# jaronlong52/neuron_poker

Hardware: AMD Instinct MI355X
Metric: Monte Carlo hand evals/sec @100k iters, 6-max preflop (higher is better)
Workload: dtype u32

## Files before the change

### neuron_poker_amd/csrc/mcq_device.hpp

```cpp
#pragma once
#include <stdint.h>

#include <algorithm>
#include <vector>

#include "../../include/mcq.h"

#if defined(__HIPCC__)
#include <hip/hip_runtime.h>
#define MCQ_HD __host__ __device__ __forceinline__
#define MCQ_HDM __host__ __device__ __forceinline__
#else
#define MCQ_HD static inline
#define MCQ_HDM inline
#endif

#define MCQ_STREAM_ITERS 16u
#define MCQ_WAVE 64u
#define MCQ_TASK_ITERS (MCQ_STREAM_ITERS * MCQ_WAVE)
#define MCQ_MAX_OPP 9

MCQ_HD uint32_t mcq_popc(uint32_t x) {
#if defined(__HIP_DEVICE_COMPILE__)
    return (uint32_t)__popc(x);
// ... 593 lines not shown
    for (uint32_t r = 0; r < MCQ_SUM_ROWS; r++) order[r] = r;
    std::stable_sort(order.begin(), order.end(), [&](uint32_t a, uint32_t b) {
        return row_lo[a + 1u] - row_lo[a] > row_lo[b + 1u] - row_lo[b];
    });
    std::vector<uint32_t> nxt(MCQ_SUM_SLOTS + 1u);
    for (uint32_t i = 0; i <= MCQ_SUM_SLOTS; i++) nxt[i] = i;
    auto next_free = [&](uint32_t i) -> uint32_t {
        while (nxt[i] != i) {
            nxt[i] = nxt[nxt[i]];
            i = nxt[i];
        }
        return i;
    };
    for (uint32_t i = 0; i < 256u; i++) t->sum.sel8[i] = t->sel8[i];
    for (uint32_t i = 0; i < MCQ_SUM_ROWS; i++) t->sum.hoff[i] = 0;
    for (uint32_t i = 0; i < MCQ_SUM_SLOTS; i++) t->sum.hrank[i] = 0;
    for (uint32_t oi = 0; oi < MCQ_SUM_ROWS && ok; oi++) {
        const uint32_t r = order[oi], lo = row_lo[r], hi = row_lo[r + 1u];
        if (lo == hi) break;
        const uint32_t col0 = MCQ_SUM_COL(ms[lo].sum), col1 = MCQ_SUM_COL(ms[hi - 1u].sum);
        uint32_t d = 0;
        for (;; d++) {
            const uint32_t at = next_free(d + col0 < MCQ_SUM_SLOTS ? d + col0 : MCQ_SUM_SLOTS);
            d = at - col0;
            if (d + col1 >= MCQ_SUM_SLOTS || d > 0xFFFFu) { ok = false; break; }
            bool fits = true;
            for (uint32_t k = lo + 1u; k < hi && fits; k++) fits = t->sum.hrank[d + MCQ_SUM_COL(ms[k].sum)] == 0u;
            if (fits) break;
        }
        if (!ok) break;
        t->sum.hoff[r] = (uint16_t)d;
        for (uint32_t k = lo; k < hi; k++) {
            const uint32_t slot = d + MCQ_SUM_COL(ms[k].sum);
            nxt[slot] = slot + 1u;
            t->sum.hrank[slot] = (uint16_t)id_of(ms[k].key);
        }
    }
    return ok;
}
static inline void mcq_fill_sum_tables(McqTables *t) { (void)mcq_fill_sum_tables_checked(t, nullptr); }

struct McqQueryCtx {
    uint32_t deck_lo, deck_hi;
    uint32_t L0;
    uint32_t n_opp;
    uint32_t n_deal;
    uint32_t runs;
    McqHole hero;
    McqBoard board;
    McqSumHole hero_s;
    McqSumBoard board_s;
};

struct McqQueryWords {
    uint32_t w0, w1, w2, w3;
    MCQ_HDM uint32_t card(uint32_t k) const {
        uint64_t v = ((uint64_t)w1 << 32) | w0;
        return (uint32_t)(v >> (8u * k)) & 0xFFu;
    }
    MCQ_HDM uint32_t n_board() const { return w1 >> 24; }
    MCQ_HDM uint32_t n_players() const { return w2 & 0xFFu; }
    MCQ_HDM uint32_t reserved() const { return w2 >> 8; }
    MCQ_HDM uint32_t runs() const { return w3; }
};

MCQ_HD bool mcq_query_valid(const McqQueryWords &q) {
    if (q.n_board() > 5 || q.n_players() < 1 || q.n_players() > 10 || q.reserved() != 0) return false;
    uint64_t seen = 0;
    bool ok = true;
    for (uint32_t i = 0; i < 2u + q.n_board(); i++) {
        uint32_t c = q.card(i);
        ok = ok && c < 52 && !((seen >> (c & 63u)) & 1);
        seen |= 1ull << (c & 63u);
    }
    return ok;
}

MCQ_HD void mcq_query_ctx(const McqQueryWords &q, McqQueryCtx &c) {
    uint64_t deck = (1ull << 52) - 1;
    c.board.clear();
    c.board_s.clear();
    for (uint32_t i = 0; i < q.n_board(); i++) {
        const uint32_t cd = q.card(2u + i);
        deck &= ~(1ull << cd);
        c.board.add(mcq_card(cd));
        c.board_s.add(mcq_card_sum(cd));
    }
    const uint32_t h0 = q.card(0), h1 = q.card(1);
    deck &= ~(1ull << h0);
    deck &= ~(1ull << h1);
    c.hero.set(mcq_card(h0), mcq_card(h1));
    c.hero_s.set(mcq_card_sum(h0), mcq_card_sum(h1));
    c.deck_lo = (uint32_t)deck;
    c.deck_hi = (uint32_t)(deck >> 32);
    c.L0 = 50u - q.n_board();
    c.n_opp = q.n_players() - 1u;
    c.n_deal = 5u - q.n_board();
    c.runs = q.runs();
}

MCQ_HD uint32_t mcq_task_weight(const McqQueryWords &q) {
    const uint32_t n = q.n_players(), deal = 5u - q.n_board();
    return 160u + 200u * n + 10u * n * n + deal * (162u - 9u * n);
}
MCQ_HD uint32_t mcq_task_count(const McqQueryWords &q) {
    return q.runs() / MCQ_TASK_ITERS + (q.runs() % MCQ_TASK_ITERS != 0u ? 1u : 0u);
}

struct McqPart {
    uint32_t t_lo, t_hi, runs;
};
MCQ_HD McqPart mcq_part(uint32_t tasks, uint32_t runs, uint32_t part, uint32_t n_parts) {
    McqPart p;
    p.t_lo = (uint32_t)((uint64_t)tasks * part / n_parts);
    p.t_hi = (uint32_t)((uint64_t)tasks * (part + 1u) / n_parts);
    const uint64_t a = (uint64_t)p.t_lo * MCQ_TASK_ITERS, b = (uint64_t)p.t_hi * MCQ_TASK_ITERS;
    p.runs = (uint32_t)((b < runs ? b : runs) - (a < runs ? a : runs));
    return p;
}

#define MCQ_SPLIT_FROM_PREP 0xFFFFFFFFu
MCQ_HD uint32_t mcq_pick_split(uint64_t total_tasks, uint64_t max_tasks, uint32_t n_cu, uint32_t split_max) {
    const uint64_t want = 8ull * n_cu;
    uint32_t s = 0;
    while (s < split_max && (total_tasks << (s + 1u)) <= want && (max_tasks << (s + 1u)) <= 512u) s++;
    return s;
}

static inline McqQueryWords mcq_query_words(const mcq_query &q) {
    McqQueryWords w;
    __builtin_memcpy(&w, &q, 16);
    return w;
}

MCQ_HD McqCard mcq_base_entry(const McqQueryCtx &qc, uint32_t l, const uint32_t *sel8) {
    uint32_t dlo = qc.deck_lo, dhi = qc.deck_hi;
    uint32_t c = mcq_select_pop(dlo, dhi, l, sel8);
    return mcq_card_sum(c < 52u ? c : 0u);
}

struct McqDeckAoS {
    const McqCard *base128;
    MCQ_HDM McqCard card(uint32_t at) const { return base128[at]; }
    MCQ_HDM McqCard hole_card(uint32_t at) const { return base128[at]; }
};
struct __attribute__((aligned(8))) McqPair {
    uint32_t a, b;
};
template <uint32_t YOFF>
struct McqDeckSplit {
    const McqPair *x128;
    MCQ_HDM McqCard card(uint32_t at) const {
        const McqPair x = x128[at], y = x128[at + YOFF];
        const McqCard c = {x.a, x.b, y.a, y.b};
        return c;
    }
    MCQ_HDM McqCard hole_card(uint32_t at) const {
        const uint32_t rb = x128[at].a;
        const McqPair y = x128[at + YOFF];
        const McqCard c = {rb, 0u, y.a, y.b};
        return c;
    }
    static MCQ_HDM void put(McqPair *x, uint32_t e, const McqCard &c) {
        const McqPair px = {c.rb, c.cnt}, py = {c.los, c.his};
        x[e] = px;
        x[e + YOFF] = py;
    }
};

struct McqLaneAcc {
    static constexpr bool kWays = false, kSeats = false;
    uint64_t types;
    uint32_t tie;
    uint32_t passes;
};
#define MCQ_N_WAYS 9u
struct McqLaneAccWays {
    static constexpr bool kWays = true, kSeats = false;
    uint64_t types;
    uint32_t passes;
    uint64_t ways;
};
#define MCQ_MAX_SEATS 10u
#define MCQ_SEAT_WIN_SHIFT 16u
#define MCQ_SEAT_TIE_SHIFT 21u
struct McqLaneAccSeats {
    static constexpr bool kWays = false, kSeats = true;
    uint32_t passes;
    uint32_t seat[MCQ_MAX_SEATS];
};
static_assert(MCQ_STREAM_ITERS * MCQ_SHARE_UNIT < (1u << MCQ_SEAT_WIN_SHIFT) && MCQ_STREAM_ITERS < 32u, "fields of McqLaneAccSeats");
MCQ_HD uint32_t mcq_seat_increment(uint32_t k) {
    static constexpr uint32_t kInc[MCQ_MAX_SEATS] = {
        2520u | (1u << MCQ_SEAT_WIN_SHIFT), 1260u | (1u << MCQ_SEAT_TIE_SHIFT), 840u | (1u << MCQ_SEAT_TIE_SHIFT),
        630u | (1u << MCQ_SEAT_TIE_SHIFT),  504u | (1u << MCQ_SEAT_TIE_SHIFT),  420u | (1u << MCQ_SEAT_TIE_SHIFT),
        360u | (1u << MCQ_SEAT_TIE_SHIFT),  315u | (1u << MCQ_SEAT_TIE_SHIFT),  280u | (1u << MCQ_SEAT_TIE_SHIFT),
        252u | (1u << MCQ_SEAT_TIE_SHIFT)};
    return kInc[k - 1u];
}

#define MCQ_HOLE_SENTINEL 0x7F7F7F7Fu

MCQ_HD void mcq_hole_reg(uint32_t rb, uint32_t &h, uint32_t &k) {
#ifdef MCQ_ABLATE_HOLES
    k += (rb ^ h) & 1u;
    return;
#endif
    const uint32_t f = ((rb - h) >> 7) & 0x01010101u;
    k = mcq_sad_u8(f, k);
    h = h + f - 0x01010101u;
}

template <int SLOT>
MCQ_HD void mcq_hole_put(uint32_t &h, uint32_t rp) {
    constexpr uint32_t sh = 8u * (SLOT & 3);
#ifdef MCQ_ABLATE_HOLES
    h = mcq_bfi(0x7Fu << sh, rp << sh, h);
    return;
#endif
    h = h + (rp << sh) - ((0x80u + 0x7Fu - (uint32_t)(SLOT & 3)) << sh);
}

MCQ_HD void mcq_hole_pair(uint32_t rp, uint32_t &h, uint32_t &k) {
    const uint32_t rp0 = h;
#ifdef MCQ_ABLATE_HOLES
    k += (rp ^ rp0) & 1u;
    h = (rp << 8) + rp0;
    return;
#endif
    const uint32_t f = rp0 <= rp ? 1u : 0u;
    k = k + f;
    const uint32_t t = mcq_opaque((rp << 8) + rp0);
    uint32_t c = MCQ_HOLE_SENTINEL - 0x01010101u - 0x7E7Eu - 0x8080u - 1u;
#if defined(__HIP_DEVICE_COMPILE__)
    asm("" : "+v"(c));
    unsigned carry_out;
    h = __builtin_addc(t, c, f, &carry_out);
#else
    h = t + c + f;
#endif
}

template <int J>
MCQ_HD uint32_t mcq_draw_opp(uint32_t rp, uint32_t (&H)[5]) {
    uint32_t k = rp;
    if (J % 4 == 1) mcq_hole_pair(rp, H[J / 4], k);
    if (J % 4 == 0) H[J / 4] = rp;
    if (J >= 2) {
        const uint32_t rb = mcq_splat_byte(rp);
#pragma unroll
        for (int i = 0; i < (J % 4 < 2 ? J / 4 : J / 4 + 1); i++) mcq_hole_reg(rb, H[i], k);
        if (J % 4 >= 2) mcq_hole_put<J>(H[J / 4], rp);
    }
    return mcq_opaque(k);
}

MCQ_HD void mcq_hole_count(uint32_t rb, uint32_t h, uint32_t &k) {
#ifdef MCQ_ABLATE_HOLES
    k += (rb ^ h) & 1u;
    return;
#endif
    k = mcq_opaque(mcq_popc((rb - h) & 0x80808080u) + k);
}

template <int K, int NREGS>
MCQ_HD uint32_t mcq_draw_table(uint32_t rp, const uint32_t (&H)[5], uint32_t &hb) {
    uint32_t p = rp;
    if (K == 0) {
        hb = rp;
    } else if (K == 1) {
        mcq_hole_pair(rp, hb, p);
    } else {
        const uint32_t rb = mcq_splat_byte(rp);
        mcq_hole_reg(rb, hb, p);
        if (K < 4) mcq_hole_put<K>(hb, rp);
    }
    uint32_t k = p;
    if (NREGS > 0) {
        const uint32_t pb = mcq_splat_byte(p);
#pragma unroll
        for (int i = 0; i < NREGS; i++) mcq_hole_count(pb, H[i], k);
    }
    return mcq_opaque(k);
}

template <int NREGS, class Draws, int NDEAL = -1, class Deck = McqDeckAoS>
MCQ_HD void mcq_deal_table(const McqQueryCtx &qc, Draws &dr, const Deck &deck, const uint32_t (&H)[5], uint32_t L,
                           McqSumBoard &b) {
    uint32_t hb = MCQ_HOLE_SENTINEL;
    const uint32_t n_deal = NDEAL >= 0 ? (uint32_t)NDEAL : mcq_opaque_uniform(qc.n_deal);
    McqCard pend = {0u, 0u, 0u, 0u};
#define MCQ_TABLE(K)                                                                                            \
    if (K < n_deal) {                                                                                           \
        const uint32_t at = mcq_draw_table<K, NREGS>(dr.template table<K>(L - Draws::kTableShort), H, hb);  \
        if (K > 0) b.add(pend);                                                                                 \
        pend = deck.card(at);                                                                                   \
        L -= 1;                                                                                                 \
    }
    MCQ_TABLE(0) MCQ_TABLE(1) MCQ_TABLE(2) MCQ_TABLE(3) MCQ_TABLE(4)
#undef MCQ_TABLE
    if (n_deal > 0u) b.add(pend);
}

MCQ_HD void mcq_join_hold(McqCard &c) {
#if defined(__HIP_DEVICE_COMPILE__)
    asm volatile("" : "+v"(c.los), "+v"(c.his));
#else
    (void)c;
#endif
}
template <class Draws, int NOPP = -1, int NDEAL = -1, class Acc = McqLaneAcc, class Deck = McqDeckAoS>
MCQ_HD void mcq_iteration_sum(const McqQueryCtx &qc, Draws &dr, const Deck &deck, const McqSumTabs &tabs, Acc &acc) {
    uint32_t H[5] = {MCQ_HOLE_SENTINEL, MCQ_HOLE_SENTINEL, MCQ_HOLE_SENTINEL, MCQ_HOLE_SENTINEL, MCQ_HOLE_SENTINEL};
    uint32_t L = qc.L0;
    McqSumHole opp[MCQ_MAX_OPP];
    const uint32_t n_opp_d = NOPP >= 0 ? (uint32_t)NOPP : mcq_opaque_uniform(qc.n_opp);
    constexpr bool kLate = NOPP >= 1;
    McqCard j1 = {0u, 0u, 0u, 0u}, j2 = {0u, 0u, 0u, 0u};
#define MCQ_OPP(P)                                                                                             \
    if (P < n_opp_d) {                                                                                         \
        uint32_t r1, r2;                                                                                       \
        dr.template pair<P>(L, r1, r2);   \
        const McqCard c1 = deck.hole_card(mcq_draw_opp<2 * P>(r1, H));               \
        const McqCard c2 = deck.hole_card(mcq_draw_opp<2 * P + 1>(r2, H));  \
        if constexpr (kLate) {                                                                                 \
            if (P > 0) {                                                                                       \
                mcq_join_hold(j2);                                                                             \
                opp[P > 0 ? P - 1 : 0].set(j1, j2);                                                            \
            }                                                                                                  \
            j1 = c1;                                                                                           \
            j2 = c2;                                                                                           \
        } else {                                                                                               \
            opp[P].set(c1, c2);                                                                                \
        }                                                                                                      \
        L -= 2;                                                                                                \
    }
    MCQ_OPP(0) MCQ_OPP(1) MCQ_OPP(2) MCQ_OPP(3) MCQ_OPP(4) MCQ_OPP(5) MCQ_OPP(6) MCQ_OPP(7) MCQ_OPP(8)
#undef MCQ_OPP
    McqSumBoard b = qc.board_s;
    if (NDEAL == 5) b.clear();
    if (NOPP >= 0) {
        mcq_deal_table<(NOPP >= 0 ? (2 * NOPP + 3) / 4 : 0), Draws, NDEAL>(qc, dr, deck, H, L, b);
    } else switch (mcq_opaque_uniform((2u * qc.n_opp + 3u) / 4u)) {
        case 0: mcq_deal_table<0, Draws>(qc, dr, deck, H, L, b); break;
        case 1: mcq_deal_table<1, Draws>(qc, dr, deck, H, L, b); break;
        case 2: mcq_deal_table<2, Draws>(qc, dr, deck, H, L, b); break;
        case 3: mcq_deal_table<3, Draws>(qc, dr, deck, H, L, b); break;
        case 4: mcq_deal_table<4, Draws>(qc, dr, deck, H, L, b); break;
        default: mcq_deal_table<5, Draws>(qc, dr, deck, H, L, b); break;
    }
    if constexpr (kLate) {
        mcq_join_hold(j2);
        opp[NOPP >= 1 ? NOPP - 1 : 0].set(j1, j2);
    }
    McqFlushSel fs;
    fs.from_board(b);
    const uint32_t hk = mcq_sum_key(b, fs, qc.hero_s, tabs);
    uint32_t best = 0;
    uint32_t n_equal = 0;
    const uint32_t n_opp_e = NOPP >= 0 ? (uint32_t)NOPP : mcq_opaque_uniform(qc.n_opp);
#define MCQ_EVAL(P)  \
    if (P < n_opp_e) {                                                     \
        uint32_t rid, fid;                                                 \
        mcq_sum_ids(b, fs, opp[P], tabs, rid, fid);                        \
        if (Acc::kWays) {  \
            const uint32_t k = rid > fid ? rid : fid;                      \
            n_equal += k == hk ? 1u : 0u;                                  \
            best = k > best ? k : best;                                    \
        } else {                                                           \
            best = mcq_max3(best, rid, fid);                               \
        }                                                                  \
    }
#ifndef MCQ_ABLATE_EVAL
    if constexpr (NOPP >= 1 && !Acc::kWays) {
        uint32_t s[MCQ_MAX_OPP], d[MCQ_MAX_OPP], fid[MCQ_MAX_OPP], rid[MCQ_MAX_OPP];
#pragma unroll
        for (int P = 0; P < NOPP; P++) mcq_sum_first(b, fs, opp[P], tabs, s[P], d[P], fid[P]);
#pragma unroll
        for (int P = 0; P < NOPP; P++) rid[P] = mcq_sum_rank(tabs, s[P], d[P]);
#pragma unroll
        for (int P = 0; P < NOPP; P++) best = mcq_max3(best, rid[P], fid[P]);
    } else
#endif
    {
        MCQ_EVAL(0) MCQ_EVAL(1) MCQ_EVAL(2) MCQ_EVAL(3) MCQ_EVAL(4) MCQ_EVAL(5) MCQ_EVAL(6) MCQ_EVAL(7) MCQ_EVAL(8)
    }
#undef MCQ_EVAL
    uint64_t won = hk >= best ? 1u : 0u;
    acc.types += won << (6u * (hk >> MCQ_ID_SHIFT));
    if constexpr (Acc::kWays) acc.ways += won << (6u * n_equal);
    else acc.tie += hk == best ? 1u : 0u;
}
template <class Draws, int NOPP = -1, int NDEAL = -1, class Acc = McqLaneAcc>
MCQ_HD void mcq_iteration(const McqQueryCtx &qc, Draws &dr, const McqCard *base128, const uint32_t *tf,
                          const uint32_t *, const uint32_t *, Acc &acc) {
    const McqDeckAoS deck = {base128};
    mcq_iteration_sum<Draws, NOPP, NDEAL, Acc>(qc, dr, deck, mcq_sum_tabs_of(tf), acc);
}

template <bool STRAIGHT, class Draws, class Acc, class Deck>
MCQ_HD void mcq_iterations_sum(const McqQueryCtx &qc, Draws &dr, const Deck &deck, const McqSumTabs &tabs, Acc &acc,
                               uint32_t cnt) {
    if (STRAIGHT) {
#define MCQ_STRAIGHT(N)                                                                                   \
    case N:                                                                                               \
        if (qc.n_deal == 5u)                                                                          \
            for (uint32_t j = 0; j < cnt; j++) mcq_iteration_sum<Draws, N, 5, Acc>(qc, dr, deck, tabs, acc); \
        else if (qc.n_deal == 2u)                                                                         \
            for (uint32_t j = 0; j < cnt; j++) mcq_iteration_sum<Draws, N, 2, Acc>(qc, dr, deck, tabs, acc); \
        else if (qc.n_deal == 1u)                                                                         \
            for (uint32_t j = 0; j < cnt; j++) mcq_iteration_sum<Draws, N, 1, Acc>(qc, dr, deck, tabs, acc); \
        else                                                                                              \
            for (uint32_t j = 0; j < cnt; j++) mcq_iteration_sum<Draws, N, -1, Acc>(qc, dr, deck, tabs, acc); \
        return;
        switch (qc.n_opp) {
            MCQ_STRAIGHT(1) MCQ_STRAIGHT(2) MCQ_STRAIGHT(3) MCQ_STRAIGHT(4) MCQ_STRAIGHT(5) MCQ_STRAIGHT(6) MCQ_STRAIGHT(7)
            case 8:
                for (uint32_t j = 0; j < cnt; j++) mcq_iteration_sum<Draws, 8, -1, Acc>(qc, dr, deck, tabs, acc);
                return;
            case 9:
                for (uint32_t j = 0; j < cnt; j++) mcq_iteration_sum<Draws, 9, -1, Acc>(qc, dr, deck, tabs, acc);
                return;
            default: break;
        }
#undef MCQ_STRAIGHT
    }
    for (uint32_t j = 0; j < cnt; j++) mcq_iteration_sum<Draws, -1, -1, Acc>(qc, dr, deck, tabs, acc);
}
template <bool STRAIGHT, class Draws, class Acc>
MCQ_HD void mcq_iterations(const McqQueryCtx &qc, Draws &dr, const McqCard *base128, const uint32_t *tf, const uint32_t *,
                           const uint32_t *, Acc &acc, uint32_t cnt) {
    const McqDeckAoS deck = {base128};
    mcq_iterations_sum<STRAIGHT>(qc, dr, deck, mcq_sum_tabs_of(tf), acc, cnt);
}

template <class Acc, class Deck>
MCQ_HD void mcq_iterations_replay4(const McqQueryCtx &qc, McqReplayDraws4 &dr, const Deck &deck, const McqSumTabs &tabs,
                                   Acc &acc, uint32_t cnt4) {
#define MCQ_REPLAY4(N)                                                                      \
    case N:                                                                                 \
        for (uint32_t k = 0; k < cnt4; k++) {                                               \
            dr.sh = 8u * k;                                                                 \
            mcq_iteration_sum<McqReplayDraws4, N, -1, Acc>(qc, dr, deck, tabs, acc);        \
        }                                                                                   \
        return;
    if constexpr (!Acc::kWays) switch (qc.n_opp) {
        MCQ_REPLAY4(1) MCQ_REPLAY4(2) MCQ_REPLAY4(3) MCQ_REPLAY4(4) MCQ_REPLAY4(5)
        default: break;
    }
#undef MCQ_REPLAY4
    for (uint32_t k = 0; k < cnt4; k++) {
        dr.sh = 8u * k;
        mcq_iteration_sum<McqReplayDraws4, -1, -1, Acc>(qc, dr, deck, tabs, acc);
    }
}

#define MCQ_EXT_WORDS 76u
#define MCQ_EXT_MAX_LISTS 11u
#define MCQ_EXT_LIST_STRIDE 2704u
#define MCQ_EXT_MAX_TRIALS 65536u

struct McqExtRec {
    const uint32_t *w;
    MCQ_HDM uint32_t ghost(uint32_t i) const { return (w[0] >> (8u * i)) & 0xFFu; }
    MCQ_HDM uint32_t hero_is_range() const { return (w[0] >> 16) & 0xFFu; }
    MCQ_HDM uint32_t n_known() const { return w[0] >> 24; }
    MCQ_HDM uint32_t known_head(uint32_t k) const { return w[13u + 7u * k]; }
    MCQ_HDM uint32_t opp_set() const { return 1u; }
    MCQ_HDM uint32_t hero_set() const { return 7u; }
    MCQ_HDM uint32_t known_set(uint32_t k) const { return 14u + 7u * k; }
};

MCQ_HD uint32_t mcq_class_index(uint32_t a, uint32_t b) {
    const uint32_t ra = a >> 2, rb = b >> 2, lo = ra < rb ? ra : rb, hi = ra < rb ? rb : ra;
    if (ra == rb) return 14u * ra;
    return (a & 3u) == (b & 3u) ? 13u * lo + hi : 13u * hi + lo;
}
MCQ_HD bool mcq_in_range(const uint32_t *bits, uint32_t a, uint32_t b) {
    const uint32_t i = mcq_class_index(a, b);
    return (bits[i >> 5] >> (i & 31u)) & 1u;
}

MCQ_HD uint32_t mcq_ext_hand(const McqQueryWords &q, const McqExtRec &e, uint32_t h) {
    if (h == 0) return e.hero_is_range() ? 0x10000u : (q.card(0) | (q.card(1) << 8));
    const uint32_t hd = e.known_head(h - 1u);
    return (hd >> 16) & 0xFFu ? 0x10000u : (hd & 0xFFFFu);
}
MCQ_HD uint32_t mcq_ext_hand_set(const McqExtRec &e, uint32_t h) { return h == 0 ? e.hero_set() : e.known_set(h - 1u); }

MCQ_HD bool mcq_ext_opp_all(const McqExtRec &e) {
    uint32_t all = e.w[e.opp_set() + 5u] | ~0x1FFu;
    for (uint32_t i = 0; i < 5; i++) all &= e.w[e.opp_set() + i];
    return all == 0xFFFFFFFFu;
}

MCQ_HD uint32_t mcq_ext_n_lists(const McqQueryWords &q, const McqExtRec &e) {
    uint32_t n = q.n_players() > 1u + e.n_known() && !mcq_ext_opp_all(e) ? 1u : 0u;
    for (uint32_t h = 0; h <= e.n_known(); h++) n += mcq_ext_hand(q, e, h) >> 16;
    return n;
}

#define MCQ_EXT_SHORT_STREAM 2u
#define MCQ_EXT_SHORT_RUNS 8192u
MCQ_HD uint32_t mcq_ext_stream_iters(const McqQueryWords &q, const McqExtRec &e) {
    return q.runs() <= MCQ_EXT_SHORT_RUNS && mcq_ext_n_lists(q, e) != 0u ? MCQ_EXT_SHORT_STREAM : MCQ_STREAM_ITERS;
}
MCQ_HD uint32_t mcq_ext_task_count(const McqQueryWords &q, uint32_t s_iters) {
    const uint32_t per = s_iters * MCQ_WAVE;
    return q.runs() / per + (q.runs() % per != 0u ? 1u : 0u);
}
MCQ_HD uint32_t mcq_ext_task_weight(const McqQueryWords &q, uint32_t s_iters) { return 3u * mcq_task_weight(q) * (s_iters >> 1); }

MCQ_HD uint64_t mcq_ext_base_deck(const McqQueryWords &q, const McqExtRec &e) {
    uint64_t deck = (1ull << 52) - 1;
    for (uint32_t i = 0; i < q.n_board(); i++) deck &= ~(1ull << q.card(2u + i));
    if (e.ghost(0) != 0xFFu) deck &= ~((1ull << e.ghost(0)) | (1ull << e.ghost(1)));
    return deck;
}

MCQ_HD void mcq_ext_list_plan(const McqQueryWords &q, const McqExtRec &e, uint32_t li, uint64_t &U, uint32_t &set_off) {
    U = mcq_ext_base_deck(q, e);
    set_off = e.opp_set();
    uint32_t seen = 0;
    for (uint32_t h = 0; h <= e.n_known(); h++) {
        const uint32_t hd = mcq_ext_hand(q, e, h);
        if (hd >> 16) {
            if (seen == li) { set_off = mcq_ext_hand_set(e, h); return; }
            seen++;
        } else {
            U &= ~((1ull << (hd & 0xFFu)) | (1ull << ((hd >> 8) & 0xFFu)));
        }
    }
}

MCQ_HD bool mcq_ext_candidate(uint64_t U, const uint32_t *set, uint32_t c) {
    const uint32_t a = c / 52u, b = c - 52u * a;
    return c < 2704u && a != b && ((U >> a) & 1u) && ((U >> b) & 1u) && mcq_in_range(set, a, b);
}

MCQ_HD bool mcq_query_ext_valid(const McqQueryWords &q, const McqExtRec &e) {
    if (q.n_board() > 5 || q.n_players() < 1 || q.n_players() > 10 || q.reserved() != 0) return false;
    if (e.hero_is_range() > 1 || e.n_known() > MCQ_MAX_KNOWN || q.n_players() < 1u + e.n_known()) return false;
    uint64_t seen = 0;
    bool ok = true;
    for (uint32_t i = 0; i < q.n_board(); i++) {
        const uint32_t c = q.card(2u + i);
        ok = ok && c < 52 && !((seen >> (c & 63u)) & 1);
        seen |= 1ull << (c & 63u);
    }
    if (e.ghost(0) != 0xFFu || e.ghost(1) != 0xFFu)
        for (uint32_t i = 0; i < 2; i++) {
            const uint32_t c = e.ghost(i);
            ok = ok && c < 52 && !((seen >> (c & 63u)) & 1);
            seen |= 1ull << (c & 63u);
        }
    for (uint32_t h = 0; h <= e.n_known(); h++) {
        if (h > 0) {
            const uint32_t hd = e.known_head(h - 1u);
            if (((hd >> 16) & 0xFFu) > 1u || (hd >> 24) != 0u) return false;
        }
        const uint32_t hd = mcq_ext_hand(q, e, h);
        if (hd >> 16) {
            const uint32_t off = mcq_ext_hand_set(e, h);
            uint32_t any = 0;
            for (uint32_t i = 0; i < 6; i++) any |= e.w[off + i];
            ok = ok && any != 0;
        } else {
            for (uint32_t i = 0; i < 2; i++) {
                const uint32_t c = (hd >> (8u * i)) & 0xFFu;
                ok = ok && c < 52 && !((seen >> (c & 63u)) & 1);
                seen |= 1ull << (c & 63u);
            }
        }
    }
    if (q.n_players() > 1u + e.n_known()) {
        uint32_t any = 0;
        for (uint32_t i = 0; i < 6; i++) any |= e.w[e.opp_set() + i];
        ok = ok && any != 0;
    }
    return ok;
}

struct McqExtCtx {
    uint32_t deck_lo, deck_hi;
    uint32_t n_players, n_hands, n_deal, runs;
    bool opp_all;
    McqBoard board;
    bool fast;
    uint32_t fdeck_lo, fdeck_hi;
    McqHole hero;
};
struct McqExtWaveCtx {
    uint32_t hand[10];
    uint32_t cnt[MCQ_EXT_MAX_LISTS];
    uint32_t pad_[3];
    const uint16_t *list[MCQ_EXT_MAX_LISTS];
};

MCQ_HD void mcq_ext_ctx(const McqQueryWords &q, const McqExtRec &e, McqExtCtx &c) {
    const uint64_t deck = mcq_ext_base_deck(q, e);
    c.board.clear();
    for (uint32_t i = 0; i < q.n_board(); i++) c.board.add(mcq_card(q.card(2u + i)));
    c.deck_lo = (uint32_t)deck;
    c.deck_hi = (uint32_t)(deck >> 32);
    c.n_players = q.n_players();
    c.n_hands = 1u + e.n_known();
    c.n_deal = 5u - q.n_board();
    c.runs = q.runs();
    c.opp_all = mcq_ext_opp_all(e);
    c.fast = !e.hero_is_range() && e.n_known() == 0u && !c.opp_all && q.n_players() >= 2u;
    const uint32_t h0 = q.card(0), h1 = q.card(1);
    const uint64_t fdeck = deck & ~(((uint64_t)1 << (h0 & 63u)) | ((uint64_t)1 << (h1 & 63u)));
    c.fdeck_lo = (uint32_t)fdeck;
    c.fdeck_hi = (uint32_t)(fdeck >> 32);
    c.hero.set(mcq_card(h0 < 52u ? h0 : 0u), mcq_card(h1 < 52u ? h1 : 0u));
}

MCQ_HD bool mcq_deck_has(uint32_t lo, uint32_t hi, uint32_t c) { return (((c & 32u) ? hi : lo) >> (c & 31u)) & 1u; }
MCQ_HD void mcq_deck_take(uint32_t &lo, uint32_t &hi, uint32_t c) {
    const uint32_t bit = 1u << (c & 31u);
    lo &= (c & 32u) ? 0xFFFFFFFFu : ~bit;
    hi &= (c & 32u) ? ~bit : 0xFFFFFFFFu;
}
MCQ_HD uint32_t mcq_deck_top(uint32_t lo, uint32_t hi) {
    return hi ? 63u - mcq_clz(hi) : 31u - mcq_clz(lo | 1u);
}
MCQ_HD uint32_t mcq_deck_next(uint32_t lo, uint32_t hi, uint32_t c) {
    const uint64_t above = ((((uint64_t)hi << 32) | lo) >> c) >> 1;
    const uint32_t alo = (uint32_t)above, ahi = (uint32_t)(above >> 32);
    const uint32_t low = alo ? alo & (0u - alo) : ahi & (0u - ahi);
    return c + 1u + (alo ? 31u - mcq_clz(low | 1u) : 63u - mcq_clz(low | 1u));
}

struct McqExtCtrDraws {
    static constexpr bool kReplay = false;
    McqStreamRng rng;
    uint32_t w;
    MCQ_HDM void start(uint64_t seed, uint64_t qid, uint32_t stream) {
        w = 0;
        rng.seed(seed, qid, stream);
    }
    MCQ_HDM uint32_t pick(uint32_t n) { return mcq_mulhi(rng.next(), n); }
    MCQ_HDM void pair(uint32_t &, uint32_t &) {}
    MCQ_HDM void index_pair(uint32_t L, uint32_t &r1, uint32_t &r2) {
// ... 214 lines not shown
```

Measured before the change: 735.7 billion.

## Plan card-draw rejection counting in compile-time epochs to cut per-draw compare work

Adds a compile-time dynamic program that splits the sequence of drawn cards into epochs and lays out held cards in packed byte registers per epoch. Each draw then adjusts its index with per-epoch counting passes, with the split chosen by an instruction-cost model, instead of the existing hole-sorted insertion scheme. When the number of opponents is known at compile time, the new planned draw path replaces the old one for both hole cards and board cards. The remaining-deck count L also becomes a compile-time constant when NDEAL is fixed. The cost model is a heuristic and may not match the real instruction count, so it can add register pressure.

After: 758.5 billion (median of 6 runs). 3.1% higher.

```diff
diff --git a/neuron_poker_amd/csrc/mcq_device.hpp b/neuron_poker_amd/csrc/mcq_device.hpp
--- a/neuron_poker_amd/csrc/mcq_device.hpp
+++ b/neuron_poker_amd/csrc/mcq_device.hpp
@@ -919,6 +919,177 @@
     if (n_deal > 0u) b.add(pend);
 }
 
+#define MCQ_DEAL_FULLREG 9
+#define MCQ_PLAN_MAX_DRAWS (2 * MCQ_MAX_OPP + 5)
+#define MCQ_PLAN_MAX_EPOCHS 6
+#define MCQ_PLAN_REGS 6
+struct McqDealPlan {
+    int n_draws, n_epochs;
+    int first[MCQ_PLAN_MAX_EPOCHS + 1];
+    int reg0[MCQ_PLAN_MAX_EPOCHS + 1];
+    constexpr int epoch_of(int d) const {
+        int e = 0;
+        while (e + 1 < n_epochs && d >= first[e + 1]) e++;
+        return e;
+    }
+    constexpr int size(int e) const { return first[e + 1] - first[e]; }
+};
+constexpr int mcq_plan_count_regs(int holes) { return holes / 4 + (holes % 4 >= 2 ? 1 : 0); }
+constexpr bool mcq_plan_lone(int holes) { return holes % 4 == 1; }
+constexpr int mcq_plan_cost_closed(int n) {
+    return (mcq_plan_count_regs(n) > 0 ? 1 + 3 * mcq_plan_count_regs(n) : 0) + (mcq_plan_lone(n) ? 2 : 0);
+}
+constexpr int mcq_plan_cost_own(int j, bool last) {
+    if (last) return mcq_plan_cost_closed(j);
+    int c = j % 4 == 1 ? 4 : 0;
+    if (j >= 2) c += 1 + 5 * (j % 4 < 2 ? j / 4 : j / 4 + 1) + (j % 4 >= 2 ? 1 : 0);
+    return c;
+}
+constexpr int mcq_plan_cost_epoch(int a, int b, int n) {
+    int c = 0;
+    for (int d = a; d < b; d++) c += mcq_plan_cost_own(d - a, d == n - 1);
+    return c + (n - b) * mcq_plan_cost_closed(b - a);
+}
+constexpr McqDealPlan mcq_deal_plan(int n, int rule) {
+    McqDealPlan pl = {};
+    pl.n_draws = n;
+    int cps[MCQ_PLAN_MAX_DRAWS + 1] = {}, n_cp = 0;
+    if (rule == MCQ_DEAL_FULLREG) {
+        for (int c = 4; c < n; c += 4) cps[n_cp++] = c;
+    } else {
+        constexpr int kInf = 1 << 28;
+        int f[MCQ_PLAN_MAX_EPOCHS + 1][MCQ_PLAN_MAX_DRAWS + 1] = {}, from[MCQ_PLAN_MAX_EPOCHS + 1][MCQ_PLAN_MAX_DRAWS + 1] = {};
+        for (int m = 0; m <= rule + 1; m++)
+            for (int b = 0; b <= n; b++) f[m][b] = m == 0 && b == 0 ? 0 : kInf;
+        for (int m = 1; m <= rule + 1; m++)
+            for (int b = 1; b <= n; b++)
+                for (int a = 0; a < b; a++) {
+                    if (f[m - 1][a] >= kInf) continue;
+                    const int c = f[m - 1][a] + mcq_plan_cost_epoch(a, b, n);
+                    if (c < f[m][b]) { f[m][b] = c; from[m][b] = a; }
+                }
+        int best = 1;
+        for (int m = 2; m <= rule + 1; m++)
+            if (f[m][n] < f[best][n]) best = m;
+        int b = n;
+        for (int m = best; m >= 1; m--) {
+            b = from[m][b];
+            if (m > 1) cps[m - 2] = b;
+        }
+        n_cp = best - 1;
+    }
+    pl.n_epochs = n_cp + 1;
+    for (int e = 1; e <= n_cp; e++) pl.first[e] = cps[e - 1];
+    pl.first[pl.n_epochs] = n;
+    for (int e = 0; e < pl.n_epochs; e++) {
+        const int holes = pl.size(e) - (e == pl.n_epochs - 1 ? 1 : 0);
+        pl.reg0[e + 1] = pl.reg0[e] + (holes + 3) / 4;
+    }
+    return pl;
+}
+constexpr int mcq_plan_cost(const McqDealPlan &pl) {
+    int c = 0;
+    for (int e = 0; e < pl.n_epochs; e++) c += mcq_plan_cost_epoch(pl.first[e], pl.first[e + 1], pl.n_draws);
+    return c;
+}
+constexpr bool mcq_plan_valid(const McqDealPlan &pl) {
+    if (pl.n_epochs < 1 || pl.n_epochs > MCQ_PLAN_MAX_EPOCHS || pl.first[0] != 0 || pl.first[pl.n_epochs] != pl.n_draws) return false;
+    for (int e = 0; e < pl.n_epochs; e++) {
+        if (pl.size(e) < 1) return false;
+        if (pl.size(e) - (e == pl.n_epochs - 1 ? 1 : 0) > 4 * (pl.reg0[e + 1] - pl.reg0[e])) return false;
+    }
+    return pl.reg0[pl.n_epochs] <= MCQ_PLAN_REGS;
+}
+template <int N, int RULE>
+struct McqPlanOf {
+    static constexpr McqDealPlan pl = mcq_deal_plan(N, RULE);
+    static_assert(mcq_plan_valid(pl), "dealing plan");
+};
+static_assert(mcq_plan_cost(mcq_deal_plan(15, 1)) == 148 && mcq_deal_plan(15, 1).first[1] == 8, "6-max before the flop, {8}");
+static_assert(mcq_plan_cost(mcq_deal_plan(15, 2)) == 145 && mcq_deal_plan(15, 2).first[2] == 12, "6-max before the flop, {8, 12}");
+static_assert(mcq_plan_cost(mcq_deal_plan(15, 3)) == 143 && mcq_deal_plan(15, 3).first[3] == 13, "6-max before the flop, {8, 12, 13}");
+static_assert(mcq_plan_cost(mcq_deal_plan(15, MCQ_DEAL_FULLREG)) == 146, "6-max before the flop, {4, 8, 12}");
+static_assert(mcq_plan_cost(mcq_deal_plan(23, 3)) == 308 && mcq_plan_cost(mcq_deal_plan(12, 3)) == 98, "ten players; 5 opponents, 2 to come");
+
+template <int N, int RULE, int EE>
+MCQ_HD void mcq_epoch_pass(const uint32_t (&E)[MCQ_PLAN_REGS], uint32_t &k) {
+    if constexpr (EE >= 0) {
+        constexpr int n = McqPlanOf<N, RULE>::pl.size(EE), r0 = McqPlanOf<N, RULE>::pl.reg0[EE];
+        const uint32_t p = k;
+        if constexpr (mcq_plan_lone(n)) k += E[r0 + n / 4] <= p ? 1u : 0u;
+        if constexpr (mcq_plan_count_regs(n) > 0) {
+            const uint32_t pb = mcq_splat_byte(p);
+#pragma unroll
+            for (int i = 0; i < mcq_plan_count_regs(n); i++) mcq_hole_count(pb, E[r0 + i], k);
+        }
+        mcq_epoch_pass<N, RULE, EE - 1>(E, k);
+    }
+}
+#if defined(__GNUC__) && !defined(__clang__)
+#define MCQ_NO_FOLD __attribute__((no_icf))
+#else
+#define MCQ_NO_FOLD
+#endif
+template <int N, int RULE, int D>
+MCQ_NO_FOLD MCQ_HD uint32_t mcq_draw_epoch(uint32_t rp, uint32_t (&E)[MCQ_PLAN_REGS]) {
+    if constexpr (D >= N) {
+        return rp;
+    } else {
+        constexpr int e = McqPlanOf<N, RULE>::pl.epoch_of(D), J = D - McqPlanOf<N, RULE>::pl.first[e],
+                      R0 = McqPlanOf<N, RULE>::pl.reg0[e];
+        uint32_t k = rp;
+        if constexpr (D == N - 1) {
+            if constexpr (mcq_plan_lone(J)) k += E[R0 + J / 4] <= rp ? 1u : 0u;
+            if constexpr (mcq_plan_count_regs(J) > 0) {
+                const uint32_t rb = mcq_splat_byte(rp);
+#pragma unroll
+                for (int i = 0; i < mcq_plan_count_regs(J); i++) mcq_hole_count(rb, E[R0 + i], k);
+            }
+        } else {
+            if constexpr (J % 4 == 1) mcq_hole_pair(rp, E[R0 + J / 4], k);
+            if constexpr (J % 4 == 0) E[R0 + J / 4] = rp;
+            if constexpr (J >= 2) {
+                const uint32_t rb = mcq_splat_byte(rp);
+#pragma unroll
+                for (int i = 0; i < (J % 4 < 2 ? J / 4 : J / 4 + 1); i++) mcq_hole_reg(rb, E[R0 + i], k);
+                if constexpr (J % 4 >= 2) mcq_hole_put<J>(E[R0 + J / 4], rp);
+            }
+        }
+        mcq_epoch_pass<N, RULE, e - 1>(E, k);
+        return mcq_opaque(k);
+    }
+}
+
+#ifndef MCQ_DEAL_RULE
+#define MCQ_DEAL_RULE 3
+#endif
+constexpr int mcq_plan_draws(int nopp, int ndeal) { return 2 * nopp + (ndeal >= 0 ? ndeal : 5); }
+
+#ifndef MCQ_L0_CONST
+#define MCQ_L0_CONST 1
+#endif
+template <int N, int RULE, int D>
+MCQ_HD uint32_t mcq_draw_opp_by(uint32_t rp, uint32_t (&H)[5], uint32_t (&E)[MCQ_PLAN_REGS]) {
+    if constexpr (RULE != 0) return mcq_draw_epoch<N, RULE, D>(rp, E);
+    else return mcq_draw_opp<D>(rp, H);
+}
+template <int N, int RULE, int D0, class Draws, int NDEAL = -1, class Deck = McqDeckAoS>
+MCQ_HD void mcq_deal_table_plan(const McqQueryCtx &qc, Draws &dr, const Deck &deck, uint32_t (&E)[MCQ_PLAN_REGS], uint32_t L,
+                                McqSumBoard &b) {
+    const uint32_t n_deal = NDEAL >= 0 ? (uint32_t)NDEAL : mcq_opaque_uniform(qc.n_deal);
+    McqCard pend = {0u, 0u, 0u, 0u};
+#define MCQ_TABLE(K)                                                                                                  \
+    if (K < n_deal) {                                                                                                 \
+        const uint32_t at = mcq_draw_epoch<N, RULE, D0 + K>(dr.template table<K>(L - Draws::kTableShort), E);  \
+        if (K > 0) b.add(pend);                                                                                       \
+        pend = deck.card(at);                                                                                         \
+        L -= 1;                                                                                                       \
+    }
+    MCQ_TABLE(0) MCQ_TABLE(1) MCQ_TABLE(2) MCQ_TABLE(3) MCQ_TABLE(4)
+#undef MCQ_TABLE
+    if (n_deal > 0u) b.add(pend);
+}
+
 MCQ_HD void mcq_join_hold(McqCard &c) {
 #if defined(__HIP_DEVICE_COMPILE__)
     asm volatile("" : "+v"(c.los), "+v"(c.his));
@@ -926,10 +1097,15 @@
     (void)c;
 #endif
 }
-template <class Draws, int NOPP = -1, int NDEAL = -1, class Acc = McqLaneAcc, class Deck = McqDeckAoS>
+template <class Draws, int NOPP = -1, int NDEAL = -1, class Acc = McqLaneAcc, class Deck = McqDeckAoS,
+          int RULE = (NOPP >= 1 ? MCQ_DEAL_RULE : 0)>
 MCQ_HD void mcq_iteration_sum(const McqQueryCtx &qc, Draws &dr, const Deck &deck, const McqSumTabs &tabs, Acc &acc) {
+    static_assert(RULE == 0 || NOPP >= 1, "a plan needs the number of opponents at compile time");
+    constexpr int kN = mcq_plan_draws(NOPP, NDEAL);
     uint32_t H[5] = {MCQ_HOLE_SENTINEL, MCQ_HOLE_SENTINEL, MCQ_HOLE_SENTINEL, MCQ_HOLE_SENTINEL, MCQ_HOLE_SENTINEL};
-    uint32_t L = qc.L0;
+    uint32_t E[MCQ_PLAN_REGS] = {MCQ_HOLE_SENTINEL, MCQ_HOLE_SENTINEL, MCQ_HOLE_SENTINEL,
+                                 MCQ_HOLE_SENTINEL, MCQ_HOLE_SENTINEL, MCQ_HOLE_SENTINEL};
+    uint32_t L = MCQ_L0_CONST && NDEAL >= 0 ? (uint32_t)(45 + NDEAL) : qc.L0;
     McqSumHole opp[MCQ_MAX_OPP];
     const uint32_t n_opp_d = NOPP >= 0 ? (uint32_t)NOPP : mcq_opaque_uniform(qc.n_opp);
     constexpr bool kLate = NOPP >= 1;
@@ -938,8 +1114,8 @@
     if (P < n_opp_d) {                                                                                         \
         uint32_t r1, r2;                                                                                       \
         dr.template pair<P>(L, r1, r2);   \
-        const McqCard c1 = deck.hole_card(mcq_draw_opp<2 * P>(r1, H));               \
-        const McqCard c2 = deck.hole_card(mcq_draw_opp<2 * P + 1>(r2, H));  \
+        const McqCard c1 = deck.hole_card(mcq_draw_opp_by<kN, RULE, 2 * P>(r1, H, E));      \
+        const McqCard c2 = deck.hole_card(mcq_draw_opp_by<kN, RULE, 2 * P + 1>(r2, H, E));  \
         if constexpr (kLate) {                                                                                 \
             if (P > 0) {                                                                                       \
                 mcq_join_hold(j2);                                                                             \
@@ -956,7 +1132,9 @@
 #undef MCQ_OPP
     McqSumBoard b = qc.board_s;
     if (NDEAL == 5) b.clear();
-    if (NOPP >= 0) {
+    if constexpr (RULE != 0) {
+        mcq_deal_table_plan<kN, RULE, 2 * NOPP, Draws, NDEAL>(qc, dr, deck, E, L, b);
+    } else if (NOPP >= 0) {
         mcq_deal_table<(NOPP >= 0 ? (2 * NOPP + 3) / 4 : 0), Draws, NDEAL>(qc, dr, deck, H, L, b);
     } else switch (mcq_opaque_uniform((2u * qc.n_opp + 3u) / 4u)) {
         case 0: mcq_deal_table<0, Draws>(qc, dr, deck, H, L, b); break;
```
